# soldasim/BOSS.jl

Hardware: AMD Instinct MI355X
Metric: gp_posterior_updates_per_sec (+ acq_evals_per_sec), N=4096 d=8 fp64 (higher is better)
Workload: dtype f64; 1 GPU; d=8 synthetic blackbox, GaussianProcess(Matern52) surrogate, N=4096 fp64 posterior update + ExpectedImprovement over 8192 candidates per GPU (BASELINE.json configs[1]+[2]); N=4096, d=8, M_per_gpu=8192, kernel=matern52, parallelism=single GPU: no exchange

## Files before the change

boss.jl_amd/api.py:

```python
from __future__ import annotations

import ctypes as C
import os
from typing import Optional, Sequence

import numpy as np

_HERE = os.path.dirname(os.path.abspath(__file__))
LIB_PATH = os.environ.get("BOSS_LIB_PATH") or os.path.join(_HERE, "libbosship.so")

BOSS_OK, BOSS_E_INVALID, BOSS_E_NO_DEVICE, BOSS_E_NOT_PD, BOSS_E_NEG_VAR, BOSS_E_NOT_FITTED, BOSS_E_ALLOC = range(7)
KERNELS = {"matern32": 0, "matern52": 1, "sqexp": 2}
FIT_NO_SYNC = 1

_c_dp = C.POINTER(C.c_double)
_c_ucp = C.POINTER(C.c_ubyte)

SIGNATURES = {
    "boss_version": (C.c_char_p, []),
    "boss_last_error": (C.c_char_p, []),
    "boss_device_count": (C.c_int, [C.POINTER(C.c_int)]),
    "boss_set_stream": (C.c_int, [C.c_int, C.c_void_p]),
    "boss_device_sync": (C.c_int, [C.c_int]),
    "boss_gp_create": (C.c_int, [C.c_int, C.c_int, C.c_int, C.c_int, _c_dp, _c_dp, _c_ucp, C.POINTER(C.c_void_p)]),
# ... 2270 lines not shown
    fn = load_library().boss_debug_acq_prune_bounds
    fn.restype = C.c_int
    fn.argtypes = [C.c_int, C.c_int, C.c_void_p, C.c_void_p, C.c_void_p]
    mua, vs, ub = np.zeros(M), np.zeros(M), np.zeros(M)
    _check(fn(device, int(M), mua.ctypes.data, vs.ctypes.data, ub.ctypes.data))
    return mua, vs, ub


def _acq_counters(g: GP):
    fn = load_library().boss_debug_acq_counters
    fn.restype = C.c_int
    fn.argtypes = [C.c_void_p, C.POINTER(C.c_long)]
    out = (C.c_long * 4)()
    _check(fn(g._h, out))
    return tuple(out)
```

boss.jl_amd/csrc/bosship.hip:

```cpp
#include "../../include/bosship.h"

#include <hip/hip_runtime.h>

#include <algorithm>
#include <cmath>
#include <cstdint>
#include <cstdio>
#include <cstdlib>
#include <atomic>
#include <chrono>
#include <cstring>
#include <functional>
#include <limits>
#include <map>
#include <mutex>
#include <string>
#include <thread>
#include <vector>

#include "gp_kernels.hpp"
#include "potrf.hpp"
#include "chain.hpp"
#include "small_calls.hpp"
#include "rider.hpp"
// ... 85 lines not shown
    long set_launches = 0, set_pre_launches = 0;
    long set_grad_launches = 0;
    bool lookahead = true;
    bool prof_on = false;
    std::map<std::string, std::vector<std::pair<hipEvent_t, hipEvent_t>>> prof;
    std::vector<hipEvent_t> ev_pool;
    Workspace vscratch, csc, pred, acq, batchA, batchX, batchMisc, craw, lgA, lgB, lgC, few, setdesc, setmom, gsetdesc, nlatjobs, mceps, meanws, warpws, prunews;
    static constexpr int LLG_BANKS = 4;
    Workspace lgbank[LLG_BANKS - 1][3];
    hipStream_t llg_stream[LLG_BANKS - 1] = {nullptr, nullptr, nullptr};
    hipEvent_t llg_join[LLG_BANKS - 1] = {nullptr, nullptr, nullptr};
    void* pinned = nullptr;
    int prune_last[5] = {0, 0, 0, 0, 0};
    long prune_launches = 0;
    int prune_M = 0;
    struct TrailTab {
        TrailWork* dev = nullptr;
        std::vector<TrailWork> host;
        std::vector<int> off;
    };
    TrailTab trail[65];
    std::mutex mtx;
};

static void chain_quiesce(Ctx* c) {
    if (c->chain_stream) (void)hipStreamSynchronize(c->chain_stream);
    if (c->strip_stream) (void)hipStreamSynchronize(c->strip_stream);
}

static std::mutex g_ctx_mtx;
// ... 155 lines not shown
                hipLaunchKernelGGL(chain_probe_wait_kernel, dim3(1), dim3(64), 0, probed[i], c->sig_panel + SIGW_NEAR + 1, 4ull, okw + i);
            int okh[4] = {0, 0, 0, 0};
            bool fine = hipDeviceSynchronize() == hipSuccess && hipMemcpy(okh, okw, sizeof okh, hipMemcpyDeviceToHost) == hipSuccess;
            (void)hipFree(okw);
            if (!(fine && okh[0] && okh[1] && okh[2] && okh[3])) c->chain_ok = false;
            if (getenv("BOSS_CHAIN_VERBOSE"))
                std::fprintf(stderr, "[bosship] resident chain: %s (main / side / chain / strip streams side by side: %d %d %d %d)\n",
                             c->chain_ok ? "on" : "off", okh[0], okh[1], okh[2], okh[3]);
        }
    }
    HIPCHK(hipHostMalloc(&c->pinned, PINNED_BYTES, hipHostMallocDefault));
    std::memset(c->pinned, 0, PINNED_UP_OFF);
    HIPCHK(hipFuncSetAttribute((const void*)potrf_diag_kernel, hipFuncAttributeMaxDynamicSharedMemorySize, DIAG_LDS_BYTES));
    HIPCHK(hipFuncSetAttribute((const void*)potrf_chain_kernel, hipFuncAttributeMaxDynamicSharedMemorySize, CHAIN_LDS_BYTES));
    HIPCHK(hipFuncSetAttribute((const void*)potrf_strips_kernel, hipFuncAttributeMaxDynamicSharedMemorySize, STRIPS_LDS_BYTES));
    {
        int cus = 0;
        if (hipDeviceGetAttribute(&cus, hipDeviceAttributeMultiprocessorCount, c->device) != hipSuccess) cus = 0;
        if (cus > 0) c->n_cus = cus;
    }
    HIPCHK(hipFuncSetAttribute((const void*)small_fit_kernel, hipFuncAttributeMaxDynamicSharedMemorySize, SMALL_LDS_BYTES));
    HIPCHK(hipFuncSetAttribute((const void*)small_llgrad_kernel, hipFuncAttributeMaxDynamicSharedMemorySize, SMALL_LLG_LDS_BYTES));
    HIPCHK(hipFuncSetAttribute((const void*)small_fit_batch_kernel, hipFuncAttributeMaxDynamicSharedMemorySize, SMALL_LDS_BYTES));
    HIPCHK(hipFuncSetAttribute((const void*)small_predict_grad_kernel<true>, hipFuncAttributeMaxDynamicSharedMemorySize, SPG_LDS_BYTES));
    HIPCHK(hipFuncSetAttribute((const void*)small_predict_grad_kernel<false>, hipFuncAttributeMaxDynamicSharedMemorySize, SPG_LDS_BYTES));
    HIPCHK(hipFuncSetAttribute((const void*)potrf_syrk_kernel<2, true>, hipFuncAttributeMaxDynamicSharedMemorySize, 96 * 1024));
    HIPCHK(hipFuncSetAttribute((const void*)rider_step_kernel, hipFuncAttributeMaxDynamicSharedMemorySize, 96 * 1024));
    HIPCHK(hipFuncSetAttribute((const void*)predict_kernel<PredG32>, hipFuncAttributeMaxDynamicSharedMemorySize,
                               PredictLds<PredG32>::BYTES));
    HIPCHK(hipFuncSetAttribute((const void*)prune_head_kernel<PredG32>, hipFuncAttributeMaxDynamicSharedMemorySize,
// ... 171 lines not shown
    int npts = 0, ldx = 0, nhead = 0;
    bool gibbs = false;
    double *lamX = nullptr, *ampX = nullptr, *noiseX = nullptr;
    double *Winv = nullptr, *Linv = nullptr;
    double* W2 = nullptr;
    int w2_np = 0;
    unsigned long long w2_gen = ~0ull;
    bool w2_used = false;
    bool have_winv = false;
    int few_calls = 0;
    int append_calls = 0;
    double* prune_a = nullptr;
    int prune_a_np = 0;
    unsigned long long prune_a_gen = ~0ull;
    int prune_skip = 0, prune_backoff = 0;
    int append_path = 0;
};

struct boss_cand {
    Ctx* ctx = nullptr;
    int d = 0, M = 0, Mp = 0;
    double* Craw = nullptr;
};

struct boss_track {
    Ctx* ctx = nullptr;
    boss_gp* gp = nullptr;
    int d = 0, M = 0, Mp = 0, tiles = 0, Ncap = 0, N = 0;
    unsigned long long epoch = 0;
    double *V = nullptr, *Csc = nullptr, *mu = nullptr, *var = nullptr, *mean = nullptr;
// ... 239 lines not shown
```

boss.jl_amd/csrc/host_prune.inc:

```

struct PruneCfg {
    int min_tiles = -1;
    int K = 64;
    int s = 1;
    int cap = 1024;
    double slack = 1.0;
};
static PruneCfg g_prune;
constexpr double PRUNE_KMU = 1.2e-4, PRUNE_KVAR = 1e-10;
constexpr size_t PRUNE_RES_OFF = 16;

static bool prune_enabled() {
    static const bool on = !(getenv("BOSS_ACQ_PRUNE") && atoi(getenv("BOSS_ACQ_PRUNE")) == 0);
    static const bool once = [] {
        if (getenv("BOSS_ACQ_PRUNE_BLOCKS")) g_prune.s = std::max(1, atoi(getenv("BOSS_ACQ_PRUNE_BLOCKS")));
        if (getenv("BOSS_ACQ_PRUNE_CAP")) g_prune.cap = std::max(0, atoi(getenv("BOSS_ACQ_PRUNE_CAP")));
        return true;
    }();
    (void)once;
    return on;
}

extern "C" int boss_debug_acq_path(int device, int* out) {
    if (!out) return fail(BOSS_E_INVALID, "out is NULL");
// ... 27 lines not shown
    if (!(scale >= 0.0)) return fail(BOSS_E_INVALID, "scale must be >= 0");
    g_prune.slack = scale;
    return BOSS_OK;
}
extern "C" int boss_debug_acq_prune_bounds(int device, int M, double* mua_out, double* vars_out, double* ub_out) {
    Ctx* c;
    int rc = get_ctx(device, &c);
    if (rc) return rc;
    std::lock_guard<std::mutex> lk(c->mtx);
    if (M < 1 || M != c->prune_M || !c->prunews.p) return fail(BOSS_E_INVALID, "no pruned attempt with that many candidates");
    HIPCHK(hipStreamSynchronize(c->stream));
    const double* base = (const double*)c->prunews.p;
    if (mua_out) HIPCHK(hipMemcpy(mua_out, base, sizeof(double) * M, hipMemcpyDeviceToHost));
    if (vars_out) HIPCHK(hipMemcpy(vars_out, base + M, sizeof(double) * M, hipMemcpyDeviceToHost));
    if (ub_out) HIPCHK(hipMemcpy(ub_out, base + 2 * (size_t)M, sizeof(double) * M, hipMemcpyDeviceToHost));
    return BOSS_OK;
}

static int prune_few_max_tiles() {
    static const int few_max_tiles = getenv("BOSS_FEW_MAX_TILES") ? atoi(getenv("BOSS_FEW_MAX_TILES")) : 128;
    return few_max_tiles;
}
static bool prune_eligible(const boss_gp* g, const boss_cand* cd, int P, int S, const EiPar& par, bool has_out, bool defer, bool has_mc,
                           const double* dpair) {
    if (!prune_enabled() || has_out || defer || dpair || has_mc || P != 1 || S != 1 || par.mode != 1) return false;
    if (g->aug || g->gibbs || g->ctx->prof_on) return false;
    static const bool no_few = getenv("BOSS_NO_FEW") && atoi(getenv("BOSS_NO_FEW"));
    const int ftiles = (cd->M + 31) / 32, few_max_tiles = prune_few_max_tiles();
    const int min_tiles = g_prune.min_tiles >= 0 ? g_prune.min_tiles : few_max_tiles;
    if (no_few || ftiles <= min_tiles || g->Np < 4 * PRED_RB || g->d > 64 || cd->d != g->d || slab_bn(cd->M, false) != 32) return false;
// ... 8 lines not shown
    for (unsigned long i = 1;; ++i) {
        if (*seq == want) {
            got = true;
            break;
        }
        if ((i & 0x3fff) == 0 && hipStreamQuery(s) != hipErrorNotReady) break;
    }
    std::atomic_thread_fence(std::memory_order_acquire);
    if (!got) {
        (void)hipStreamSynchronize(s);
        got = *seq == want;
    }
    return got;
}

static int prune_avec(boss_gp* g, hipStream_t s, const double** a_out, bool* rebuilt) {
    *rebuilt = false;
    if (g->have_lt && g->avec) {
        *a_out = g->avec;
        return BOSS_OK;
    }
    if (g->prune_a && g->prune_a_np != g->Np) {
        (void)hipStreamSynchronize(s);
        (void)hipFree(g->prune_a);
        g->prune_a = nullptr;
    }
    if (!g->prune_a) {
        if (dev_malloc((void**)&g->prune_a, sizeof(double) * 2 * (size_t)g->Np) != hipSuccess) {
            g->prune_a = nullptr;
            return fail(BOSS_E_ALLOC, "device allocation failed");
        }
        g->prune_a_np = g->Np;
        g->prune_a_gen = ~0ull;
    }
    if (g->prune_a_gen != g->factor_gen) {
        const int nb = g->Np / PRED_RB;
        for (int ib = nb - 1; ib >= 0; --ib)
            hipLaunchKernelGGL(prune_avec_step_kernel, dim3(std::max(1, 2 * ib)), dim3(PRUNE_AVEC_THREADS), 0, s, (const double*)g->A, g->ld, g->Np, g->N,
                               (const double*)g->Dinv2, ib, ib == nb - 1 ? 1 : 0, g->prune_a + g->Np, g->prune_a);
        g->prune_a_gen = g->factor_gen;
        *rebuilt = true;
    }
    *a_out = g->prune_a;
    return BOSS_OK;
}

static int acq_prune_try(boss_gp* g, const boss_cand* cd, const double* mean_dev, const unsigned char* mask_dev, const EiPar& par,
                         bool* done, double* res_out, long* idx_out) {
    *done = false;
    Ctx* c = g->ctx;
    hipStream_t s = c->stream;
    int* last = c->prune_last;
    last[0] = 0;
    last[1] = last[2] = last[4] = 0;
    last[3] = g_prune.s;
    if (g->prune_skip > 0) {
// ... 22 lines not shown
    double* icraw = imean + nint;
    double* tpair = icraw + (size_t)d * nint;
    int* sel = (int*)(tpair + 2);
    int* surv = sel + nint;
    unsigned char* insel = (unsigned char*)(surv + M);
    c->prune_M = M;
    double* res = (double*)c->pinned + PRUNE_RES_OFF;

    if (!g->have_dinv) {
        dinv_join(g);
        dinv_launch(g, s);
        g->have_dinv = true;
    }
    dinv_join(g);
    g->dinv_used = true;
    const double* avec = nullptr;
    bool rebuilt = false;
    rc = prune_avec(g, s, &avec, &rebuilt);
    if (rc) return rc;
    last[4] = rebuilt ? 1 : 0;
    c->prune_launches += (rebuilt ? Np / PRED_RB : 0) + 7;
    double* Csc = (double*)c->csc.p;
    hipLaunchKernelGGL(scale_cand_kernel, dim3((Mp + 255) / 256), dim3(256), 0, s, cd->Craw, Csc, g->invlam, g->discrete_dev, d, Mp);
    typedef PredG32 G;
    hipLaunchKernelGGL(prune_head_kernel<G>, dim3(tiles), dim3(G::NTHREADS), PredictLds<G>::BYTES, s, (const double*)g->A, g->ld, Np, g->N,
                       (const double*)g->Dinv2, (const double*)g->Xsc, (const double*)Csc, d, Mp, g->kernel, g->amp2, (double*)c->vscratch.p, M,
                       sblk, vars);
    const size_t mu_lds = sizeof(double) * ((size_t)d + 1) * PRUNE_MU_STAGE;
    auto mu_fn = d <= 16 ? prune_mu_kernel<true> : prune_mu_kernel<false>;
    hipLaunchKernelGGL(mu_fn, dim3((M + PRUNE_MU_CANDS - 1) / PRUNE_MU_CANDS, nch), dim3(256), mu_lds, s, (const double*)g->Xsc, Np, g->N, (const double*)Csc, d, Mp, M,
                       g->kernel, g->amp2, avec, part);
    PrunePar pp;
    pp.coef = par.coefs[0];
    pp.best = par.best;
    pp.amp2 = g->amp2;
    pp.kmu = PRUNE_KMU * g_prune.slack;
    pp.kvar = PRUNE_KVAR * g_prune.slack;
    hipLaunchKernelGGL(prune_bound_kernel, dim3((M + 255) / 256), dim3(256), 0, s, (const double*)part, nch, mean_dev, (const double*)vars, mask_dev, M,
                       pp, mua, ub, keys);
    hipLaunchKernelGGL(prune_select_kernel, dim3(1), dim3(PRUNE_THREADS), 0, s, (const unsigned long long*)keys, M, K, sel, insel);

    boss_cand icd;
    icd.ctx = c;
    icd.d = d;
    auto finish_exact = [&](const int* list, int n) -> int {
        icd.M = n;
        icd.Mp = round_up(n, 64);
        icd.Craw = icraw;
        hipLaunchKernelGGL(prune_gather_kernel, dim3((icd.Mp + 255) / 256), dim3(256), 0, s, list, n, (const double*)cd->Craw, Mp, d, mean_dev,
                           icraw, icd.Mp, mean_dev ? imean : (double*)nullptr);
        return predict_enqueue(g, &icd, mean_dev ? imean : nullptr, imu, ivar, false, nullptr, nullptr, false, true);
    };
    rc = finish_exact(sel, K);
    if (rc) return drain(c, rc);
    unsigned long long seq = ++c->acq_seq;
    hipLaunchKernelGGL(prune_decide_kernel, dim3(1), dim3(PRUNE_THREADS), 0, s, (const int*)sel, K, (const double*)imu, (const double*)ivar,
                       (const double*)mua, mask_dev, par, pp, M, (const double*)ub, (const unsigned char*)insel, surv, tpair, res, seq);
    bool ok = prune_poll(c, s, res, seq);
    hipError_t e = hipGetLastError();
    if (!ok || e != hipSuccess) return fail(BOSS_E_NO_DEVICE, e != hipSuccess ? hipGetErrorString(e) : "the pruned acquisition did not report");
    long cnt = reinterpret_cast<const long*>(res)[2], bad = reinterpret_cast<const long*>(res)[3];
    last[1] = K;
    last[2] = (int)std::min<long>(cnt, 0x7fffffff);
    if (!bad && cnt > 0 && cnt <= cap) {
        rc = finish_exact(surv, (int)cnt);
        if (rc) return drain(c, rc);
        c->prune_launches += 2;
        seq = ++c->acq_seq;
        hipLaunchKernelGGL(prune_merge_kernel, dim3(1), dim3(PRUNE_THREADS), 0, s, (const int*)surv, (int)cnt, (const double*)imu,
                           (const double*)ivar, (const double*)mua, mask_dev, par, pp, (const double*)tpair, res, seq);
        ok = prune_poll(c, s, res, seq);
        e = hipGetLastError();
        if (!ok || e != hipSuccess) return fail(BOSS_E_NO_DEVICE, e != hipSuccess ? hipGetErrorString(e) : "the pruned acquisition did not report");
        bad = reinterpret_cast<const long*>(res)[3];
    }
    if (bad || cnt > cap) {
        g->prune_backoff = g->prune_backoff ? std::min(64, 2 * g->prune_backoff) : 1;
        g->prune_skip = g->prune_backoff;
        last[0] = 2;
        return BOSS_OK;
    }
    g->prune_backoff = 0;
    last[0] = 1;
    *res_out = res[0];
    *idx_out = reinterpret_cast<const long*>(res)[1];
    *done = true;
    return BOSS_OK;
}
```

boss.jl_amd/csrc/prune_kernels.hpp:

```cpp
#pragma once
#include "acq_kernels.hpp"

namespace boss {

template <int NC>
__device__ __forceinline__ void prune_wave_sums(double (&v)[NC], int lane) {
#pragma unroll
    for (int h = NC / 2; h >= 1; h >>= 1) {
        const bool up = (lane & h) != 0;
#pragma unroll
        for (int j = 0; j < h; ++j) {
            const double keep = up ? v[j + h] : v[j], send = up ? v[j] : v[j + h];
            v[j] = keep + __shfl_xor(send, h);
        }
    }
#pragma unroll
    for (int off = NC; off < 64; off <<= 1) v[0] += __shfl_xor(v[0], off);
}
constexpr int PRUNE_AVEC_THREADS = 1024;
__global__ __launch_bounds__(PRUNE_AVEC_THREADS) void prune_avec_step_kernel(const double* __restrict__ A, int ld, int Np, int N,
                                                                             const double* __restrict__ Dinv2, int ib, int first,
                                                                             double* __restrict__ r, double* __restrict__ a) {
    __shared__ double rv[PRED_RB], av[PRED_RB];
    const int tid = threadIdx.x, lane = tid & 63;
    const int wave = __builtin_amdgcn_readfirstlane(tid >> 6);
    const int i0 = ib * PRED_RB;
    if (tid < PRED_RB) {
        const int i = i0 + tid;
        rv[tid] = first ? (i < N ? A[(size_t)i * ld + Np] : 0.0) : r[i];
    }
    __syncthreads();
    const double* D = Dinv2 + (size_t)ib * PRED_RB * PRED_RB;
    double r4[4];
#pragma unroll
    for (int q = 0; q < 4; ++q) r4[q] = rv[lane + 64 * q];
    {
        double sums[16];
#pragma unroll
        for (int j = 0; j < 16; ++j) {
            const int c = 16 * j + wave;
            const double* col = D + (size_t)c * PRED_RB;
            double sacc = 0.0;
#pragma unroll
            for (int q = 0; q < 4; ++q) {
                if (q >= j / 4) {
                    const int row = lane + 64 * q;
                    const double dv = col[row];
                    sacc = __builtin_fma(row >= c ? dv : 0.0, r4[q], sacc);
                }
            }
            sums[j] = sacc;
        }
        prune_wave_sums<16>(sums, lane);
        if (lane < 16) av[16 * lane + wave] = sums[0];
    }
    __syncthreads();
    if (blockIdx.x == 0 && tid < PRED_RB) a[i0 + tid] = av[tid];
    if (ib == 0) return;
    double a4[4];
#pragma unroll
    for (int q = 0; q < 4; ++q) a4[q] = av[lane + 64 * q];
    double sums[8];
    const int cg0 = blockIdx.x * 128 + wave * 8;
#pragma unroll
    for (int j = 0; j < 8; ++j) {
        const double* col = A + (size_t)(cg0 + j) * ld + i0;
        double sacc = 0.0;
#pragma unroll
        for (int q = 0; q < 4; ++q) sacc = __builtin_fma(col[lane + 64 * q], a4[q], sacc);
        sums[j] = sacc;
    }
    prune_wave_sums<8>(sums, lane);
    if (lane < 8) {
        const int cg = cg0 + lane;
        const double base = first ? (cg < N ? A[(size_t)cg * ld + Np] : 0.0) : r[cg];
        r[cg] = base - sums[0];
    }
}

template <class G>
__global__ __launch_bounds__(G::NTHREADS) __attribute__((amdgpu_waves_per_eu(1, 1))) void prune_head_kernel(
    const double* __restrict__ A, int ld, int Np, int N, const double* __restrict__ Dinv, const double* __restrict__ Xsc,
    const double* __restrict__ Csc, int d, int Mp, int kern, double amp2, double* __restrict__ Vscratch, int M, int sblk,
    double* __restrict__ var_out) {
    static_assert(G::WC == 1 && G::BM == 2 * BLK && G::PM == 2 && G::WR == 4, "written for the 256-row, 32-candidate geometry");
    constexpr int RB = G::BM;
    extern __shared__ double lds[];
    constexpr int BN = G::BN, TM = G::TM, TN = G::TN, LDR = PredictLds<G>::LDR;
    double* Rs = lds;
    double* red = Rs + RB * LDR;
    const int tid = threadIdx.x, lane = tid & 63;
    const int wave = __builtin_amdgcn_readfirstlane(tid >> 6);
// ... 238 lines not shown
__global__ __launch_bounds__(256) void prune_bound_kernel(const double* __restrict__ part, int nch, const double* __restrict__ mean_s,
                                                          const double* __restrict__ var_s, const unsigned char* __restrict__ mask, int M,
                                                          PrunePar pp, double* __restrict__ mua, double* __restrict__ ub,
                                                          unsigned long long* __restrict__ keys) {
    const int j = blockIdx.x * 256 + threadIdx.x;
    if (j >= M) return;
    double m = mean_s ? mean_s[j] : 0.0;
    for (int ch = 0; ch < nch; ++ch) m += part[(size_t)ch * M + j];
    mua[j] = m;
    const double u = (mask && !mask[j]) ? 0.0 : prune_bound(pp, m, var_s[j]);
    ub[j] = u;
    keys[j] = prune_key(u);
}

__device__ __forceinline__ void prune_hist_add(int* hist, int bin, bool active, int lane) {
    unsigned long long todo = __ballot(active);
    while (todo) {
        const int leader = __ffsll((long long)todo) - 1;
        const int b = __shfl(bin, leader);
        const unsigned long long same = __ballot(active && bin == b);
        if (lane == leader) atomicAdd(&hist[b], (int)__popcll(same));
        todo &= ~same;
    }
}

constexpr int PRUNE_CPT_MAX = 16;
__global__ __launch_bounds__(PRUNE_THREADS) void prune_select_kernel(const unsigned long long* __restrict__ keys, int M, int K,
                                                                     int* __restrict__ sel, unsigned char* __restrict__ insel) {
    __shared__ int hist[256];
    __shared__ int scan[PRUNE_THREADS];
    __shared__ unsigned long long s_prefix;
    __shared__ int s_remaining;
    const int t = threadIdx.x, lane = t & 63;
    unsigned long long kreg[PRUNE_CPT_MAX];
#pragma unroll
    for (int i = 0; i < PRUNE_CPT_MAX; ++i) {
        const int j = t + PRUNE_THREADS * i;
        kreg[i] = j < M ? keys[j] : 0ull;
    }
    if (t == 0) {
        s_prefix = 0ull;
        s_remaining = K;
    }
    __syncthreads();
    for (int pass = 7; pass >= 0; --pass) {
        if (t < 256) hist[t] = 0;
        __syncthreads();
        const unsigned long long prefix = s_prefix;
        const int sh = 8 * pass;
#pragma unroll
        for (int i = 0; i < PRUNE_CPT_MAX; ++i) {
            const unsigned long long k = kreg[i];
            const bool in = (t + PRUNE_THREADS * i < M) && (pass == 7 || (k >> (sh + 8)) == (prefix >> (sh + 8)));
            prune_hist_add(hist, (int)((k >> sh) & 255ull), in, lane);
        }
        __syncthreads();
        const int rem = s_remaining;
        int suf = t < 256 ? hist[t] : 0;
        for (int off = 1; off < 256; off <<= 1) {
            const int add = (t < 256 && t + off < 256) ? hist[t + off] : 0;
            __syncthreads();
            if (t < 256) {
                suf += add;
                hist[t] = suf;
            }
            __syncthreads();
        }
        const int above = (t < 255) ? hist[t + 1] : 0;
        __syncthreads();
        if (t < 256 && suf >= rem && above < rem) {
            s_remaining = rem - above;
            s_prefix = prefix | ((unsigned long long)t << sh);
        }
        __syncthreads();
    }
    const unsigned long long kth = s_prefix;
    const int want_eq = s_remaining;
    const int cpt = (M + PRUNE_THREADS - 1) / PRUNE_THREADS;
    const int j0 = t * cpt, j1 = min(M, j0 + cpt);
    int ngt = 0, neq = 0;
    for (int j = j0; j < j1; ++j) {
        const unsigned long long k = keys[j];
        ngt += k > kth;
        neq += k == kth;
    }
    int tot_gt, tot_eq;
    const int eq_off = prune_exscan(neq, scan, &tot_eq);
    int take = 0, eqr = eq_off;
    for (int j = j0; j < j1; ++j) {
        const unsigned long long k = keys[j];
        if (k > kth) ++take;
        else if (k == kth) {
            if (eqr < want_eq) ++take;
            ++eqr;
        }
    }
    (void)ngt;
    const int off = prune_exscan(take, scan, &tot_gt);
    int o = off;
    eqr = eq_off;
    for (int j = j0; j < j1; ++j) {
        const unsigned long long k = keys[j];
        bool in = k > kth;
        if (k == kth) {
            in = eqr < want_eq;
            ++eqr;
        }
        insel[j] = in ? 1 : 0;
        if (in) {
            if (o < K) sel[o] = j;
            ++o;
        }
    }
}

__global__ __launch_bounds__(256) void prune_gather_kernel(const int* __restrict__ list, int n, const double* __restrict__ Craw, int Mp,
                                                           int d, const double* __restrict__ mean_s, double* __restrict__ Cint, int Mpi,
                                                           double* __restrict__ mean_int) {
    const int i = blockIdx.x * 256 + threadIdx.x;
    if (i >= Mpi) return;
    const int j = i < n ? list[i] : -1;
    for (int k = 0; k < d; ++k) Cint[(size_t)k * Mpi + i] = j >= 0 ? Craw[(size_t)k * Mp + j] : 0.0;
    if (mean_int) mean_int[i] = (j >= 0 && mean_s) ? mean_s[j] : 0.0;
}

__device__ __forceinline__ void prune_exact_reduce(const int* __restrict__ list, int n, const double* __restrict__ imu,
                                                   const double* __restrict__ ivar, const double* __restrict__ mua,
                                                   const unsigned char* __restrict__ mask, const EiPar& par, const PrunePar& pp,
// ... 32 lines not shown
    __syncthreads();
}

__device__ __forceinline__ bool prune_survives(double u, double T, long iT, long j, bool masked) {
    if (!masked && T < 2.2250738585072014e-308) u += 64 * 4.9406564584124654e-324;
    if (u < T) return false;
    if (u > T || u != u || j < iT) return true;
    return !(masked || T >= 2.2250738585072014e-308);
}

__global__ __launch_bounds__(PRUNE_THREADS) void prune_decide_kernel(const int* __restrict__ sel, int K, const double* __restrict__ imu,
                                                                     const double* __restrict__ ivar, const double* __restrict__ mua,
                                                                     const unsigned char* __restrict__ mask, EiPar par, PrunePar pp, int M,
                                                                     const double* __restrict__ ub, const unsigned char* __restrict__ insel,
                                                                     int* __restrict__ surv, double* __restrict__ tpair,
                                                                     double* __restrict__ res, unsigned long long res_seq) {
    __shared__ double sv[PRUNE_THREADS];
    __shared__ long si[PRUNE_THREADS];
    __shared__ int scan[PRUNE_THREADS];
    __shared__ int bad;
    const int t = threadIdx.x;
    if (t == 0) bad = 0;
    __syncthreads();
    double T;
    long iT;
    prune_exact_reduce(sel, K, imu, ivar, mua, mask, par, pp, sv, si, T, iT, &bad);
    const int cpt = (M + PRUNE_THREADS - 1) / PRUNE_THREADS;
    const int j0 = t * cpt, j1 = min(M, j0 + cpt);
    int cnt = 0;
    for (int j = j0; j < j1; ++j) cnt += (!insel[j] && prune_survives(ub[j], T, iT, j, mask && !mask[j])) ? 1 : 0;
    int total;
    int o = prune_exscan(cnt, scan, &total);
    for (int j = j0; j < j1; ++j)
        if (!insel[j] && prune_survives(ub[j], T, iT, j, mask && !mask[j])) surv[o++] = j;
    if (t == 0) {
        tpair[0] = T;
        reinterpret_cast<long*>(tpair)[1] = iT;
        res[0] = T;
        reinterpret_cast<long*>(res)[1] = iT;
        reinterpret_cast<long*>(res)[2] = total;
        reinterpret_cast<long*>(res)[3] = bad;
        __threadfence_system();
        __hip_atomic_store(reinterpret_cast<unsigned long long*>(res) + 4, res_seq, __ATOMIC_RELAXED, __HIP_MEMORY_SCOPE_SYSTEM);
    }
}

__global__ __launch_bounds__(PRUNE_THREADS) void prune_merge_kernel(const int* __restrict__ surv, int n, const double* __restrict__ imu,
                                                                    const double* __restrict__ ivar, const double* __restrict__ mua,
                                                                    const unsigned char* __restrict__ mask, EiPar par, PrunePar pp,
                                                                    const double* __restrict__ tpair, double* __restrict__ res,
                                                                    unsigned long long res_seq) {
    __shared__ double sv[PRUNE_THREADS];
    __shared__ long si[PRUNE_THREADS];
    __shared__ int bad;
    if (threadIdx.x == 0) bad = 0;
    __syncthreads();
// ... 21 lines not shown
```

Before: 910.6 updates/s.

## Build L^-T z in one resident kernel, fork head onto side stream, faster top-K select

The per-block chain of prune_avec_step launches (one per 256-row block) is replaced by a single persistent kernel whose blocks wait on device flags, when the grid fits on the CUs. The candidate scaling and prune head now run on the side stream in parallel with that build. prune_select_kernel is rewritten to skip radix passes whose bytes are uniform, to use wave-level scans instead of block-wide shared-memory scans, and to keep keys in registers. A give-up path detects a stalled resident wait, falls back to per-step launches and redoes the step, and debug hooks are added for testing.

```diff
diff --git a/boss.jl_amd/api.py b/boss.jl_amd/api.py
--- a/boss.jl_amd/api.py
+++ b/boss.jl_amd/api.py
@@ -2308,3 +2308,38 @@
     out = (C.c_long * 4)()
     _check(fn(g._h, out))
     return tuple(out)
+
+
+def _acq_avec(g: GP):
+    fn = load_library().boss_debug_acq_avec
+    fn.restype = C.c_int
+    fn.argtypes = [C.c_void_p, C.POINTER(C.c_long)]
+    out = (C.c_long * 2)()
+    _check(fn(g._h, out))
+    return tuple(out)
+
+
+def _acq_avec_set(g: GP, resident: int = -1):
+    fn = load_library().boss_debug_acq_avec_set
+    fn.restype = C.c_int
+    fn.argtypes = [C.c_void_p, C.c_int]
+    _check(fn(g._h, int(resident)))
+
+
+def _acq_avec_giveup(g: GP):
+    fn = load_library().boss_debug_acq_avec_giveup
+    fn.restype = C.c_int
+    fn.argtypes = [C.c_void_p]
+    _check(fn(g._h))
+
+
+def _acq_select(keys, K: int, device: int = 0):
+    keys = np.ascontiguousarray(np.asarray(keys, dtype=np.uint64))
+    Mk = keys.shape[0]
+    fn = load_library().boss_debug_acq_select
+    fn.restype = C.c_int
+    fn.argtypes = [C.c_int, C.c_void_p, C.c_int, C.c_int, C.c_void_p, C.c_void_p]
+    sel = np.zeros(int(K), dtype=np.int32)
+    insel = np.zeros(Mk, dtype=np.uint8)
+    _check(fn(device, keys.ctypes.data, Mk, int(K), sel.ctypes.data, insel.ctypes.data))
+    return sel, insel
diff --git a/boss.jl_amd/csrc/bosship.hip b/boss.jl_amd/csrc/bosship.hip
--- a/boss.jl_amd/csrc/bosship.hip
+++ b/boss.jl_amd/csrc/bosship.hip
@@ -123,6 +123,7 @@
     int prune_last[5] = {0, 0, 0, 0, 0};
     long prune_launches = 0;
     int prune_M = 0;
+    bool avec_resident_off = false;
     struct TrailTab {
         TrailWork* dev = nullptr;
         std::vector<TrailWork> host;
@@ -308,6 +309,7 @@
     HIPCHK(hipFuncSetAttribute((const void*)potrf_diag_kernel, hipFuncAttributeMaxDynamicSharedMemorySize, DIAG_LDS_BYTES));
     HIPCHK(hipFuncSetAttribute((const void*)potrf_chain_kernel, hipFuncAttributeMaxDynamicSharedMemorySize, CHAIN_LDS_BYTES));
     HIPCHK(hipFuncSetAttribute((const void*)potrf_strips_kernel, hipFuncAttributeMaxDynamicSharedMemorySize, STRIPS_LDS_BYTES));
+    HIPCHK(hipFuncSetAttribute((const void*)prune_avec_chain_kernel, hipFuncAttributeMaxDynamicSharedMemorySize, AVEC_CHAIN_LDS_BYTES));
     {
         int cus = 0;
         if (hipDeviceGetAttribute(&cus, hipDeviceAttributeMultiprocessorCount, c->device) != hipSuccess) cus = 0;
@@ -509,6 +511,8 @@
     int prune_a_np = 0;
     unsigned long long prune_a_gen = ~0ull;
     int prune_skip = 0, prune_backoff = 0;
+    bool prune_a_resident = false;
+    unsigned long long prune_a_seq = 0;
     int append_path = 0;
 };
 
diff --git a/boss.jl_amd/csrc/host_prune.inc b/boss.jl_amd/csrc/host_prune.inc
--- a/boss.jl_amd/csrc/host_prune.inc
+++ b/boss.jl_amd/csrc/host_prune.inc
@@ -65,6 +65,32 @@
     if (mua_out) HIPCHK(hipMemcpy(mua_out, base, sizeof(double) * M, hipMemcpyDeviceToHost));
     if (vars_out) HIPCHK(hipMemcpy(vars_out, base + M, sizeof(double) * M, hipMemcpyDeviceToHost));
     if (ub_out) HIPCHK(hipMemcpy(ub_out, base + 2 * (size_t)M, sizeof(double) * M, hipMemcpyDeviceToHost));
+    return BOSS_OK;
+}
+
+extern "C" int boss_debug_acq_select(int device, const unsigned long long* keys, int M, int K, int* sel_out, unsigned char* insel_out) {
+    if (!keys || !sel_out || !insel_out) return fail(BOSS_E_INVALID, "NULL argument");
+    if (K < 1 || K > M || M > PRUNE_THREADS * PRUNE_CPT_MAX) return fail(BOSS_E_INVALID, "needs 1 <= K <= M <= 16384");
+    Ctx* c;
+    int rc = get_ctx(device, &c);
+    if (rc) return rc;
+    HIPCHK(hipSetDevice(c->device));
+    std::lock_guard<std::mutex> lk(c->mtx);
+    const size_t kb = sizeof(unsigned long long) * (size_t)M, sb = sizeof(int) * (size_t)K;
+    rc = ws_reserve(c->prunews, kb + sb + (size_t)M);
+    if (rc) return rc;
+    c->prune_M = 0;
+    unsigned long long* dk = (unsigned long long*)c->prunews.p;
+    int* dsel = (int*)(dk + M);
+    unsigned char* din = (unsigned char*)(dsel + K);
+    HIPCHK(hipStreamSynchronize(c->stream));
+    HIPCHK(hipMemcpy(dk, keys, kb, hipMemcpyHostToDevice));
+    HIPCHK(hipMemsetAsync(dsel, 0xff, sb, c->stream));
+    hipLaunchKernelGGL(prune_select_kernel, dim3(1), dim3(PRUNE_THREADS), 0, c->stream, (const unsigned long long*)dk, M, K, dsel, din);
+    HIPCHK(hipGetLastError());
+    HIPCHK(hipStreamSynchronize(c->stream));
+    HIPCHK(hipMemcpy(sel_out, dsel, sb, hipMemcpyDeviceToHost));
+    HIPCHK(hipMemcpy(insel_out, din, (size_t)M, hipMemcpyDeviceToHost));
     return BOSS_OK;
 }
 
@@ -103,9 +129,70 @@
     return got;
 }
 
-static int prune_avec(boss_gp* g, hipStream_t s, const double** a_out, bool* rebuilt) {
-    *rebuilt = false;
+static int g_avec_resident = -1;
+static bool avec_fork_on() {
+    static const bool env = !(getenv("BOSS_ACQ_AVEC_FORK") && atoi(getenv("BOSS_ACQ_AVEC_FORK")) == 0);
+    return env;
+}
+static bool avec_resident_on(const boss_gp* g) {
+    static const bool env = !(getenv("BOSS_ACQ_AVEC_RESIDENT") && atoi(getenv("BOSS_ACQ_AVEC_RESIDENT")) == 0);
+    if (g->ctx->avec_resident_off || avec_chain_grid(g->Np / PRED_RB) > g->ctx->n_cus) return false;
+    return g_avec_resident < 0 ? env : g_avec_resident != 0;
+}
+static unsigned long long* prune_words(const boss_gp* g) { return reinterpret_cast<unsigned long long*>(g->prune_a + 2 * (size_t)g->Np); }
+static unsigned long long* prune_status_word(const boss_gp* g) {
+    return prune_words(g) + (size_t)(AVEC_SLICES + 1) * (g->Np / PRED_RB) * AVEC_WORD_STRIDE;
+}
+
+static void prune_avec_enqueue(boss_gp* g, hipStream_t s) {
+    const int nb = g->Np / PRED_RB;
+    double* a = g->prune_a;
+    g->prune_a_resident = avec_resident_on(g);
+    if (g->prune_a_resident) {
+        hipLaunchKernelGGL(prune_avec_chain_kernel, dim3(avec_chain_grid(nb)), dim3(AVEC_CHAIN_THREADS), AVEC_CHAIN_LDS_BYTES, s, (const double*)g->A, g->ld,
+                           g->Np, g->N, (const double*)g->Dinv2, nb, a + g->Np, a, prune_words(g), ++g->prune_a_seq, poll_budget_ticks(g->Np));
+    } else {
+        for (int ib = nb - 1; ib >= 0; --ib)
+            hipLaunchKernelGGL(prune_avec_step_kernel, dim3(std::max(1, 2 * ib)), dim3(PRUNE_AVEC_THREADS), 0, s, (const double*)g->A, g->ld, g->Np, g->N,
+                               (const double*)g->Dinv2, ib, ib == nb - 1 ? 1 : 0, a + g->Np, a);
+    }
+    g->prune_a_gen = g->factor_gen;
+}
+static int prune_avec_launches(const boss_gp* g) { return g->prune_a_resident ? 1 : g->Np / PRED_RB; }
+
+extern "C" int boss_debug_acq_avec(const boss_gp* g, long* out) {
+    if (!g || !out) return fail(BOSS_E_INVALID, "NULL argument");
+    std::lock_guard<std::mutex> lk(g->ctx->mtx);
+    out[0] = avec_resident_on(g) ? 1 : 0;
+    out[1] = (g->prune_a && g->prune_a_gen == g->factor_gen && g->prune_a_resident) ? 1 : 0;
+    return BOSS_OK;
+}
+extern "C" int boss_debug_acq_avec_set(boss_gp* g, int resident) {
+    if (!g) return fail(BOSS_E_INVALID, "gp is NULL");
+    std::lock_guard<std::mutex> lk(g->ctx->mtx);
+    if (resident != -1) g_avec_resident = resident < -1 ? -1 : resident;
+    if (resident == 1) g->ctx->avec_resident_off = false;
+    g->prune_a_gen = ~0ull;
+    return BOSS_OK;
+}
+extern "C" int boss_debug_acq_avec_giveup(boss_gp* g) {
+    if (!g) return fail(BOSS_E_INVALID, "gp is NULL");
+    Ctx* c = g->ctx;
+    HIPCHK(hipSetDevice(c->device));
+    std::lock_guard<std::mutex> lk(c->mtx);
+    if (!g->prune_a || g->prune_a_np != g->Np || g->prune_a_gen != g->factor_gen || !g->prune_a_resident)
+        return fail(BOSS_E_INVALID, "the handle has no current a from the resident build");
+    HIPCHK(hipStreamSynchronize(c->stream));
+    const unsigned long long v = g->prune_a_seq;
+    HIPCHK(hipMemcpy(prune_status_word(g), &v, sizeof v, hipMemcpyHostToDevice));
+    return BOSS_OK;
+}
+
+template <class Fork>
+static int prune_avec(boss_gp* g, hipStream_t s, const double** a_out, int* launches, Fork&& fork) {
+    *launches = 0;
     if (g->have_lt && g->avec) {
+        fork(false);
         *a_out = g->avec;
         return BOSS_OK;
     }
@@ -115,20 +202,20 @@
         g->prune_a = nullptr;
     }
     if (!g->prune_a) {
-        if (dev_malloc((void**)&g->prune_a, sizeof(double) * 2 * (size_t)g->Np) != hipSuccess) {
+        const size_t bytes = sizeof(double) * 2 * (size_t)g->Np + sizeof(unsigned long long) * avec_chain_words(g->Np / PRED_RB);
+        if (dev_malloc((void**)&g->prune_a, bytes) != hipSuccess) {
             g->prune_a = nullptr;
             return fail(BOSS_E_ALLOC, "device allocation failed");
         }
+        HIPCHK(hipMemsetAsync(g->prune_a, 0, bytes, s));
         g->prune_a_np = g->Np;
         g->prune_a_gen = ~0ull;
     }
-    if (g->prune_a_gen != g->factor_gen) {
-        const int nb = g->Np / PRED_RB;
-        for (int ib = nb - 1; ib >= 0; --ib)
-            hipLaunchKernelGGL(prune_avec_step_kernel, dim3(std::max(1, 2 * ib)), dim3(PRUNE_AVEC_THREADS), 0, s, (const double*)g->A, g->ld, g->Np, g->N,
-                               (const double*)g->Dinv2, ib, ib == nb - 1 ? 1 : 0, g->prune_a + g->Np, g->prune_a);
-        g->prune_a_gen = g->factor_gen;
-        *rebuilt = true;
+    const bool build = g->prune_a_gen != g->factor_gen;
+    fork(build);
+    if (build) {
+        prune_avec_enqueue(g, s);
+        *launches = prune_avec_launches(g);
     }
     *a_out = g->prune_a;
     return BOSS_OK;
@@ -181,18 +268,39 @@
     }
     dinv_join(g);
     g->dinv_used = true;
+    double* Csc = (double*)c->csc.p;
+    typedef PredG32 G;
+    auto head = [&](hipStream_t hs) {
+        hipLaunchKernelGGL(scale_cand_kernel, dim3((Mp + 255) / 256), dim3(256), 0, hs, cd->Craw, Csc, g->invlam, g->discrete_dev, d, Mp);
+        hipLaunchKernelGGL(prune_head_kernel<G>, dim3(tiles), dim3(G::NTHREADS), PredictLds<G>::BYTES, hs, (const double*)g->A, g->ld, Np, g->N,
+                           (const double*)g->Dinv2, (const double*)g->Xsc, (const double*)Csc, d, Mp, g->kernel, g->amp2,
+                           (double*)c->vscratch.p, M, sblk, vars);
+    };
+    hipEvent_t ev_join = nullptr;
+    auto fork = [&](bool build) {
+        if (build && avec_fork_on()) {
+            if (!c->ev_pool.empty()) {
+                ev_join = c->ev_pool.back();
+                c->ev_pool.pop_back();
+            } else if (hipEventCreate(&ev_join) != hipSuccess) ev_join = nullptr;
+        }
+        if (!ev_join) return head(s);
+        (void)hipEventRecord(c->ev_fork, s);
+        (void)hipStreamWaitEvent(c->side_stream, c->ev_fork, 0);
+        head(c->side_stream);
+        (void)hipEventRecord(ev_join, c->side_stream);
+    };
     const double* avec = nullptr;
-    bool rebuilt = false;
-    rc = prune_avec(g, s, &avec, &rebuilt);
-    if (rc) return rc;
-    last[4] = rebuilt ? 1 : 0;
-    c->prune_launches += (rebuilt ? Np / PRED_RB : 0) + 7;
-    double* Csc = (double*)c->csc.p;
-    hipLaunchKernelGGL(scale_cand_kernel, dim3((Mp + 255) / 256), dim3(256), 0, s, cd->Craw, Csc, g->invlam, g->discrete_dev, d, Mp);
-    typedef PredG32 G;
-    hipLaunchKernelGGL(prune_head_kernel<G>, dim3(tiles), dim3(G::NTHREADS), PredictLds<G>::BYTES, s, (const double*)g->A, g->ld, Np, g->N,
-                       (const double*)g->Dinv2, (const double*)g->Xsc, (const double*)Csc, d, Mp, g->kernel, g->amp2, (double*)c->vscratch.p, M,
-                       sblk, vars);
+    int built = 0;
+    rc = prune_avec(g, s, &avec, &built, fork);
+    if (ev_join) {
+        (void)hipStreamWaitEvent(s, ev_join, 0);
+        c->ev_pool.push_back(ev_join);
+    }
+    if (rc) return rc;
+    last[4] = built ? 1 : 0;
+    c->prune_launches += built + 7;
+    const bool a_resident = avec == g->prune_a && g->prune_a_resident;
     const size_t mu_lds = sizeof(double) * ((size_t)d + 1) * PRUNE_MU_STAGE;
     auto mu_fn = d <= 16 ? prune_mu_kernel<true> : prune_mu_kernel<false>;
     hipLaunchKernelGGL(mu_fn, dim3((M + PRUNE_MU_CANDS - 1) / PRUNE_MU_CANDS, nch), dim3(256), mu_lds, s, (const double*)g->Xsc, Np, g->N, (const double*)Csc, d, Mp, M,
@@ -222,7 +330,8 @@
     if (rc) return drain(c, rc);
     unsigned long long seq = ++c->acq_seq;
     hipLaunchKernelGGL(prune_decide_kernel, dim3(1), dim3(PRUNE_THREADS), 0, s, (const int*)sel, K, (const double*)imu, (const double*)ivar,
-                       (const double*)mua, mask_dev, par, pp, M, (const double*)ub, (const unsigned char*)insel, surv, tpair, res, seq);
+                       (const double*)mua, mask_dev, par, pp, M, (const double*)ub, (const unsigned char*)insel, surv, tpair, res, seq,
+                       a_resident ? (const unsigned long long*)prune_status_word(g) : (const unsigned long long*)nullptr, g->prune_a_seq);
     bool ok = prune_poll(c, s, res, seq);
     hipError_t e = hipGetLastError();
     if (!ok || e != hipSuccess) return fail(BOSS_E_NO_DEVICE, e != hipSuccess ? hipGetErrorString(e) : "the pruned acquisition did not report");
@@ -241,6 +350,16 @@
         if (!ok || e != hipSuccess) return fail(BOSS_E_NO_DEVICE, e != hipSuccess ? hipGetErrorString(e) : "the pruned acquisition did not report");
         bad = reinterpret_cast<const long*>(res)[3];
     }
+    if (bad & 2) {
+        static std::atomic<int> warned{0};
+        if (warned.fetch_add(1) < 2 && !getenv("BOSS_QUIET"))
+            std::fprintf(stderr, "[bosship] device %d: a wait inside the resident build of L^-T z gave up — built by one launch per step from now on "
+                         "(results are unaffected)\n", c->device);
+        c->avec_resident_off = true;
+        g->prune_a_gen = ~0ull;
+        last[0] = 2;
+        return BOSS_OK;
+    }
     if (bad || cnt > cap) {
         g->prune_backoff = g->prune_backoff ? std::min(64, 2 * g->prune_backoff) : 1;
         g->prune_skip = g->prune_backoff;
diff --git a/boss.jl_amd/csrc/prune_kernels.hpp b/boss.jl_amd/csrc/prune_kernels.hpp
--- a/boss.jl_amd/csrc/prune_kernels.hpp
+++ b/boss.jl_amd/csrc/prune_kernels.hpp
@@ -17,6 +17,54 @@
 #pragma unroll
     for (int off = NC; off < 64; off <<= 1) v[0] += __shfl_xor(v[0], off);
 }
+__device__ __forceinline__ void prune_dinv_load(const double* __restrict__ D, int role, int lane, double (&dv)[16][4]) {
+#pragma unroll
+    for (int j = 0; j < 16; ++j) {
+        const double* col = D + (size_t)(16 * j + role) * PRED_RB;
+#pragma unroll
+        for (int q = 0; q < 4; ++q)
+            if (q >= j / 4) dv[j][q] = col[lane + 64 * q];
+    }
+}
+__device__ __forceinline__ double prune_dinv_dot(const double (&dv)[16][4], const double (&r4)[4], int role, int lane) {
+    double sums[16];
+#pragma unroll
+    for (int j = 0; j < 16; ++j) {
+        const int c = 16 * j + role;
+        double sacc = 0.0;
+#pragma unroll
+        for (int q = 0; q < 4; ++q) {
+            if (q >= j / 4) {
+                const int row = lane + 64 * q;
+                sacc = __builtin_fma(row >= c ? dv[j][q] : 0.0, r4[q], sacc);
+            }
+        }
+        sums[j] = sacc;
+    }
+    prune_wave_sums<16>(sums, lane);
+    return sums[0];
+}
+__device__ __forceinline__ void prune_lcol_load(const double* __restrict__ A, int ld, int cg0, int i0, int lane, double (&lv)[8][4]) {
+#pragma unroll
+    for (int j = 0; j < 8; ++j) {
+        const double* col = A + (size_t)(cg0 + j) * ld + i0;
+#pragma unroll
+        for (int q = 0; q < 4; ++q) lv[j][q] = col[lane + 64 * q];
+    }
+}
+__device__ __forceinline__ double prune_lcol_dot(const double (&lv)[8][4], const double (&a4)[4], int lane) {
+    double sums[8];
+#pragma unroll
+    for (int j = 0; j < 8; ++j) {
+        double sacc = 0.0;
+#pragma unroll
+        for (int q = 0; q < 4; ++q) sacc = __builtin_fma(lv[j][q], a4[q], sacc);
+        sums[j] = sacc;
+    }
+    prune_wave_sums<8>(sums, lane);
+    return sums[0];
+}
+
 constexpr int PRUNE_AVEC_THREADS = 1024;
 __global__ __launch_bounds__(PRUNE_AVEC_THREADS) void prune_avec_step_kernel(const double* __restrict__ A, int ld, int Np, int N,
                                                                              const double* __restrict__ Dinv2, int ib, int first,
@@ -35,24 +83,10 @@
 #pragma unroll
     for (int q = 0; q < 4; ++q) r4[q] = rv[lane + 64 * q];
     {
-        double sums[16];
-#pragma unroll
-        for (int j = 0; j < 16; ++j) {
-            const int c = 16 * j + wave;
-            const double* col = D + (size_t)c * PRED_RB;
-            double sacc = 0.0;
-#pragma unroll
-            for (int q = 0; q < 4; ++q) {
-                if (q >= j / 4) {
-                    const int row = lane + 64 * q;
-                    const double dv = col[row];
-                    sacc = __builtin_fma(row >= c ? dv : 0.0, r4[q], sacc);
-                }
-            }
-            sums[j] = sacc;
-        }
-        prune_wave_sums<16>(sums, lane);
-        if (lane < 16) av[16 * lane + wave] = sums[0];
+        double dv[16][4];
+        prune_dinv_load(D, wave, lane, dv);
+        const double s = prune_dinv_dot(dv, r4, wave, lane);
+        if (lane < 16) av[16 * lane + wave] = s;
     }
     __syncthreads();
     if (blockIdx.x == 0 && tid < PRED_RB) a[i0 + tid] = av[tid];
@@ -60,22 +94,118 @@
     double a4[4];
 #pragma unroll
     for (int q = 0; q < 4; ++q) a4[q] = av[lane + 64 * q];
-    double sums[8];
     const int cg0 = blockIdx.x * 128 + wave * 8;
-#pragma unroll
-    for (int j = 0; j < 8; ++j) {
-        const double* col = A + (size_t)(cg0 + j) * ld + i0;
-        double sacc = 0.0;
-#pragma unroll
-        for (int q = 0; q < 4; ++q) sacc = __builtin_fma(col[lane + 64 * q], a4[q], sacc);
-        sums[j] = sacc;
-    }
-    prune_wave_sums<8>(sums, lane);
+    double lv[8][4];
+    prune_lcol_load(A, ld, cg0, i0, lane, lv);
+    const double s = prune_lcol_dot(lv, a4, lane);
     if (lane < 8) {
         const int cg = cg0 + lane;
         const double base = first ? (cg < N ? A[(size_t)cg * ld + Np] : 0.0) : r[cg];
-        r[cg] = base - sums[0];
-    }
+        r[cg] = base - s;
+    }
+}
+
+constexpr int AVEC_CHAIN_THREADS = 512, AVEC_SLICE = 64, AVEC_SLICES = PRED_RB / AVEC_SLICE, AVEC_WORD_STRIDE = 16;
+constexpr int AVEC_CHAIN_LDS_BYTES = 90 * 1024;
+__host__ __device__ constexpr int avec_chain_grid(int nb) { return 1 + (AVEC_SLICES + 1) * (nb - 1); }
+__host__ __device__ constexpr int avec_chain_words(int nb) { return ((AVEC_SLICES + 1) * nb + 1) * AVEC_WORD_STRIDE; }
+__device__ __forceinline__ bool avec_wait(const unsigned long long* w, int nw, unsigned long long seq, unsigned long long* status,
+                                          unsigned budget, int lane) {
+    const PollTimer tm(budget);
+    for (int it = 0; it < POLL_CAP; ++it) {
+        const unsigned long long v = lane < nw ? ld_word(w + (size_t)lane * AVEC_WORD_STRIDE) : ~0ull;
+        if (__all(v >= seq)) {
+            asm volatile("" ::: "memory");
+            return true;
+        }
+        if ((it & 63) == 63) {
+            if (ld_word(status) >= seq) return false;
+            if (tm.expired()) break;
+        }
+        __builtin_amdgcn_s_sleep(1);
+    }
+    if (lane == 0) raise_word(status, seq);
+    return false;
+}
+__global__ __launch_bounds__(AVEC_CHAIN_THREADS) void prune_avec_chain_kernel(const double* __restrict__ A, int ld, int Np, int N,
+                                                                              const double* __restrict__ Dinv2, int nb, double* r, double* a,
+                                                                              unsigned long long* words, unsigned long long seq,
+                                                                              unsigned budget) {
+    __shared__ double av[PRED_RB];
+    __shared__ int s_ok;
+    const int tid = threadIdx.x, lane = tid & 63;
+    const int wave = __builtin_amdgcn_readfirstlane(tid >> 6);
+    const int b = blockIdx.x;
+    const int per = AVEC_SLICES + 1;
+    const int jb = b == 0 ? nb - 1 : nb - 2 - (b - 1) / per;
+    const int role = b == 0 ? AVEC_SLICES : (b - 1) % per;
+    unsigned long long* status = words + (size_t)per * nb * AVEC_WORD_STRIDE;
+    unsigned long long* wj = words + (size_t)per * jb * AVEC_WORD_STRIDE;
+    if (tid == 0) s_ok = 1;
+    __syncthreads();
+    if (role < AVEC_SLICES) {
+        const int cg0 = jb * PRED_RB + role * AVEC_SLICE + wave * 8;
+        const int cg = cg0 + (lane & 7);
+        double res = cg < N ? A[(size_t)cg * ld + Np] : 0.0;
+        double lv[8][4];
+        prune_lcol_load(A, ld, cg0, (nb - 1) * PRED_RB, lane, lv);
+        for (int i = nb - 1; i > jb; --i) {
+            double nx[8][4];
+            if (i - 1 > jb) prune_lcol_load(A, ld, cg0, (i - 1) * PRED_RB, lane, nx);
+            if (wave == 0 && *(volatile int*)&s_ok) {
+                const bool ok = avec_wait(words + ((size_t)per * i + AVEC_SLICES) * AVEC_WORD_STRIDE, 1, seq, status, budget, lane);
+                if (!ok && lane == 0) *(volatile int*)&s_ok = 0;
+            }
+            __syncthreads();
+            double a4[4];
+#pragma unroll
+            for (int q = 0; q < 4; ++q) a4[q] = ld_sc1(a + (size_t)i * PRED_RB + lane + 64 * q);
+            const double s = prune_lcol_dot(lv, a4, lane);
+            res = res - s;
+            if (i - 1 > jb) {
+#pragma unroll
+                for (int j = 0; j < 8; ++j)
+#pragma unroll
+                    for (int q = 0; q < 4; ++q) lv[j][q] = nx[j][q];
+            }
+        }
+        if (lane < 8) st_sc1(r + cg, res);
+        drain_stores();
+        __syncthreads();
+        if (tid == 0) raise_word(wj + (size_t)role * AVEC_WORD_STRIDE, seq);
+        return;
+    }
+    const double* D = Dinv2 + (size_t)jb * PRED_RB * PRED_RB;
+    double d0[16][4], d1[16][4];
+    prune_dinv_load(D, wave, lane, d0);
+    prune_dinv_load(D, wave + 8, lane, d1);
+    double r4[4];
+    if (jb == nb - 1) {
+#pragma unroll
+        for (int q = 0; q < 4; ++q) {
+            const int i = jb * PRED_RB + lane + 64 * q;
+            r4[q] = i < N ? A[(size_t)i * ld + Np] : 0.0;
+        }
+    } else {
+        if (wave == 0) {
+            const bool ok = avec_wait(wj, AVEC_SLICES, seq, status, budget, lane);
+            if (!ok && lane == 0) *(volatile int*)&s_ok = 0;
+        }
+        __syncthreads();
+#pragma unroll
+        for (int q = 0; q < 4; ++q) r4[q] = ld_sc1(r + (size_t)jb * PRED_RB + lane + 64 * q);
+    }
+    const double s0 = prune_dinv_dot(d0, r4, wave, lane);
+    const double s1 = prune_dinv_dot(d1, r4, wave + 8, lane);
+    if (lane < 16) {
+        av[16 * lane + wave] = s0;
+        av[16 * lane + wave + 8] = s1;
+    }
+    __syncthreads();
+    if (tid < PRED_RB) st_sc1(a + (size_t)jb * PRED_RB + tid, av[tid]);
+    drain_stores();
+    __syncthreads();
+    if (tid == 0) raise_word(wj + (size_t)AVEC_SLICES * AVEC_WORD_STRIDE, seq);
 }
 
 template <class G>
@@ -344,104 +474,141 @@
 }
 
 __device__ __forceinline__ void prune_hist_add(int* hist, int bin, bool active, int lane) {
-    unsigned long long todo = __ballot(active);
-    while (todo) {
-        const int leader = __ffsll((long long)todo) - 1;
-        const int b = __shfl(bin, leader);
-        const unsigned long long same = __ballot(active && bin == b);
-        if (lane == leader) atomicAdd(&hist[b], (int)__popcll(same));
-        todo &= ~same;
-    }
+    const unsigned long long todo = __ballot(active);
+    if (!todo) return;
+    const int leader = __ffsll((long long)todo) - 1;
+    const int b = __shfl(bin, leader);
+    const unsigned long long same = __ballot(active && bin == b);
+    if (lane == leader) atomicAdd(&hist[b], (int)__popcll(same));
+    else if (active && bin != b) atomicAdd(&hist[bin], 1);
 }
 
 constexpr int PRUNE_CPT_MAX = 16;
 __global__ __launch_bounds__(PRUNE_THREADS) void prune_select_kernel(const unsigned long long* __restrict__ keys, int M, int K,
                                                                      int* __restrict__ sel, unsigned char* __restrict__ insel) {
+    constexpr int NW = PRUNE_THREADS / 64;
     __shared__ int hist[256];
-    __shared__ int scan[PRUNE_THREADS];
+    __shared__ int wtot[NW];
+    __shared__ unsigned long long w_and[NW], w_or[NW];
     __shared__ unsigned long long s_prefix;
     __shared__ int s_remaining;
-    const int t = threadIdx.x, lane = t & 63;
+    const int t = threadIdx.x, lane = t & 63, wave = t >> 6;
     unsigned long long kreg[PRUNE_CPT_MAX];
 #pragma unroll
     for (int i = 0; i < PRUNE_CPT_MAX; ++i) {
         const int j = t + PRUNE_THREADS * i;
         kreg[i] = j < M ? keys[j] : 0ull;
     }
-    if (t == 0) {
-        s_prefix = 0ull;
-        s_remaining = K;
-    }
-    __syncthreads();
-    for (int pass = 7; pass >= 0; --pass) {
-        if (t < 256) hist[t] = 0;
-        __syncthreads();
-        const unsigned long long prefix = s_prefix;
-        const int sh = 8 * pass;
+    const int cpt = (M + PRUNE_THREADS - 1) / PRUNE_THREADS;
+    const int j0 = t * cpt, j1 = min(M, j0 + cpt);
+    unsigned long long kc[PRUNE_CPT_MAX];
+#pragma unroll
+    for (int i = 0; i < PRUNE_CPT_MAX; ++i) kc[i] = j0 + i < j1 ? keys[j0 + i] : 0ull;
+    unsigned long long prefix = 0ull;
+    int rem = K;
+    int fixed = 64;
+    while (fixed > 0) {
+        unsigned long long va = ~0ull, vo = 0ull;
+        unsigned live = 0u;
 #pragma unroll
         for (int i = 0; i < PRUNE_CPT_MAX; ++i) {
             const unsigned long long k = kreg[i];
-            const bool in = (t + PRUNE_THREADS * i < M) && (pass == 7 || (k >> (sh + 8)) == (prefix >> (sh + 8)));
-            prune_hist_add(hist, (int)((k >> sh) & 255ull), in, lane);
-        }
-        __syncthreads();
-        const int rem = s_remaining;
-        int suf = t < 256 ? hist[t] : 0;
-        for (int off = 1; off < 256; off <<= 1) {
-            const int add = (t < 256 && t + off < 256) ? hist[t + off] : 0;
-            __syncthreads();
-            if (t < 256) {
-                suf += add;
-                hist[t] = suf;
-            }
-            __syncthreads();
-        }
-        const int above = (t < 255) ? hist[t + 1] : 0;
-        __syncthreads();
-        if (t < 256 && suf >= rem && above < rem) {
-            s_remaining = rem - above;
-            s_prefix = prefix | ((unsigned long long)t << sh);
-        }
-        __syncthreads();
-    }
-    const unsigned long long kth = s_prefix;
-    const int want_eq = s_remaining;
-    const int cpt = (M + PRUNE_THREADS - 1) / PRUNE_THREADS;
-    const int j0 = t * cpt, j1 = min(M, j0 + cpt);
+            const bool in = (t + PRUNE_THREADS * i < M) && (fixed == 64 || (k >> fixed) == (prefix >> fixed));
+            if (in) {
+                va &= k;
+                vo |= k;
+                live |= 1u << i;
+            }
+        }
+#pragma unroll
+        for (int off = 32; off >= 1; off >>= 1) {
+            va &= __shfl_xor(va, off);
+            vo |= __shfl_xor(vo, off);
+        }
+        if (lane == 0) {
+            w_and[wave] = va;
+            w_or[wave] = vo;
+        }
+        __syncthreads();
+        va = ~0ull;
+        vo = 0ull;
+#pragma unroll
+        for (int w = 0; w < NW; ++w) {
+            va &= w_and[w];
+            vo |= w_or[w];
+        }
+        const unsigned long long diff = va ^ vo;
+        if (diff == 0ull) {
+            prefix = va;
+            break;
+        }
+        const int sh = 8 * ((63 - __clzll((long long)diff)) >> 3);
+        prefix = sh + 8 < 64 ? (va >> (sh + 8)) << (sh + 8) : 0ull;
+        if (t < 256) hist[t] = 0;
+        __syncthreads();
+#pragma unroll
+        for (int i = 0; i < PRUNE_CPT_MAX; ++i) prune_hist_add(hist, (int)((kreg[i] >> sh) & 255ull), (live >> i) & 1u, lane);
+        __syncthreads();
+        const int own = t < 256 ? hist[t] : 0;
+        int suf = own;
+#pragma unroll
+        for (int off = 1; off < 64; off <<= 1) {
+            const int u = __shfl_down(suf, off);
+            if (lane + off < 64) suf += u;
+        }
+        if (t < 256 && lane == 0) wtot[wave] = suf;
+        __syncthreads();
+        if (t < 256) {
+            for (int w = wave + 1; w < 4; ++w) suf += wtot[w];
+            const int above = suf - own;
+            if (suf >= rem && above < rem) {
+                s_remaining = rem - above;
+                s_prefix = prefix | ((unsigned long long)t << sh);
+            }
+        }
+        __syncthreads();
+        prefix = s_prefix;
+        rem = s_remaining;
+        fixed = sh;
+    }
+    const unsigned long long kth = prefix;
+    const int want_eq = rem;
     int ngt = 0, neq = 0;
-    for (int j = j0; j < j1; ++j) {
-        const unsigned long long k = keys[j];
-        ngt += k > kth;
-        neq += k == kth;
-    }
-    int tot_gt, tot_eq;
-    const int eq_off = prune_exscan(neq, scan, &tot_eq);
-    int take = 0, eqr = eq_off;
-    for (int j = j0; j < j1; ++j) {
-        const unsigned long long k = keys[j];
-        if (k > kth) ++take;
-        else if (k == kth) {
-            if (eqr < want_eq) ++take;
-            ++eqr;
-        }
-    }
-    (void)ngt;
-    const int off = prune_exscan(take, scan, &tot_gt);
-    int o = off;
-    eqr = eq_off;
-    for (int j = j0; j < j1; ++j) {
-        const unsigned long long k = keys[j];
-        bool in = k > kth;
-        if (k == kth) {
-            in = eqr < want_eq;
-            ++eqr;
-        }
-        insel[j] = in ? 1 : 0;
-        if (in) {
-            if (o < K) sel[o] = j;
-            ++o;
-        }
-    }
+#pragma unroll
+    for (int i = 0; i < PRUNE_CPT_MAX; ++i)
+        if (j0 + i < j1) {
+            ngt += kc[i] > kth;
+            neq += kc[i] == kth;
+        }
+    const int packed = ngt | (neq << 16);
+    int incl = packed;
+#pragma unroll
+    for (int off = 1; off < 64; off <<= 1) {
+        const int u = __shfl_up(incl, off);
+        if (lane >= off) incl += u;
+    }
+    if (lane == 63) wtot[wave] = incl;
+    __syncthreads();
+    int excl = incl - packed;
+    for (int w = 0; w < wave; ++w) excl += wtot[w];
+    const int eq_off = excl >> 16;
+    int o = (excl & 0xffff) + min(eq_off, want_eq);
+    int eqr = eq_off;
+#pragma unroll
+    for (int i = 0; i < PRUNE_CPT_MAX; ++i)
+        if (j0 + i < j1) {
+            const unsigned long long k = kc[i];
+            bool in = k > kth;
+            if (k == kth) {
+                in = eqr < want_eq;
+                ++eqr;
+            }
+            insel[j0 + i] = in ? 1 : 0;
+            if (in) {
+                if (o < K) sel[o] = j0 + i;
+                ++o;
+            }
+        }
 }
 
 __global__ __launch_bounds__(256) void prune_gather_kernel(const int* __restrict__ list, int n, const double* __restrict__ Craw, int Mp,
@@ -504,7 +671,8 @@
                                                                      const unsigned char* __restrict__ mask, EiPar par, PrunePar pp, int M,
                                                                      const double* __restrict__ ub, const unsigned char* __restrict__ insel,
                                                                      int* __restrict__ surv, double* __restrict__ tpair,
-                                                                     double* __restrict__ res, unsigned long long res_seq) {
+                                                                     double* __restrict__ res, unsigned long long res_seq,
+                                                                     const unsigned long long* st_word, unsigned long long st_seq) {
     __shared__ double sv[PRUNE_THREADS];
     __shared__ long si[PRUNE_THREADS];
     __shared__ int scan[PRUNE_THREADS];
@@ -529,7 +697,7 @@
         res[0] = T;
         reinterpret_cast<long*>(res)[1] = iT;
         reinterpret_cast<long*>(res)[2] = total;
-        reinterpret_cast<long*>(res)[3] = bad;
+        reinterpret_cast<long*>(res)[3] = bad | ((st_word && ld_word(st_word) >= st_seq) ? 2 : 0);
         __threadfence_system();
         __hip_atomic_store(reinterpret_cast<unsigned long long*>(res) + 4, res_seq, __ATOMIC_RELAXED, __HIP_MEMORY_SCOPE_SYSTEM);
     }
```

Measured after the change: 915.4 updates/s (median of 6 runs). About the same (+0.5%).
